# MustaphaMensouri/Distributed-Continuous-Training-with-Airflow-PyTorch-Distributed-DDP-

Measured on AMD Instinct MI355X. Metric: samples/sec (whole node) for weather-MLP DDP, higher is better.
Workload: dtype fp32; 1 GPU; global_batch=4, per_rank_batch=4, parallelism=dp1, optimizer=adam lr=0.01, loss=ce, engine=fused-persistent, dataset_rows=8649, features=5

## Files before the change

### distributed-continuous-training-with-airflow-pytorch-distributed-ddp-_amd/csrc/mlp_block5.hip

```cpp
#include "knobs.h"
#include "mlp_block5_impl.h"

namespace dct {

void mlp_launch_block5_xg(int world, size_t bytes, hipStream_t st, const MlpShape& sh, const MlpArgs& a);
void mlp_launch_block5_b8(size_t bytes, hipStream_t st, const MlpShape& sh, const MlpArgs& a);

static bool b5_xg_world_ok(int w) { return w >= 2 && w <= 8; }

bool mlp_block5_ok(const MlpShape& sh, const MlpArgs& a) {
  const bool aligned = (sh.woff[1] % 4) == 0 && ((uintptr_t)a.p & 15) == 0 && (((uintptr_t)a.m | (uintptr_t)a.v) & 15) == 0;
  const bool xg_ok = a.xg_world <= 1 ||
                     (a.mode == 0 && b5_xg_world_ok(a.xg_world) && a.xg_rank >= 0 && a.xg_rank < a.xg_world &&
                      a.xg_recv != nullptr && a.xg_peers != nullptr && a.xg_status != nullptr &&
                      (a.prof == nullptr || a.xg_world == 2 || a.xg_world == 4 || a.xg_world == 8));
  const bool b8_ok = (a.B <= blk5::B && sh.mlp_block != 8) || a.prof == nullptr;
  return aligned && b8_ok && mlp_block5_shape_ok(sh.dims, sh.L, a.B) &&
         ((a.mode == 0 && a.cursor == nullptr) || (a.mode == 1 && a.steps == 1 && a.grad_out != nullptr)) &&
         (a.loss_kind == 0 || a.loss_kind == 1) && a.pending == nullptr && (a.stage == nullptr || a.mode == 1) && xg_ok;
}

bool mlp_block5_shape_ok(const int* dims, int L, int B) {
  return L == 3 && dims[1] == blk5::H && dims[2] == blk5::H && dims[0] >= 1 && dims[0] <= blk5::DMAX &&
         dims[3] == blk5::C && B >= 1 && B <= blk5::BMAX;
}

size_t mlp_block5_xg_bytes(int world) {
  switch (world) {
    case 2: return (size_t)b5x::Lay<2>::BYTES;
    case 4: return (size_t)b5x::Lay<4>::BYTES;
    case 8: return (size_t)b5x::Lay<8>::BYTES;
    case 3: return (size_t)b5x::Lay<3>::BYTES;
    case 5: return (size_t)b5x::Lay<5>::BYTES;
    case 6: return (size_t)b5x::Lay<6>::BYTES;
    case 7: return (size_t)b5x::Lay<7>::BYTES;
    default: return 0;
  }
}

template <bool WD, int LK, bool PROF = false>
static void b5_launch_sched(int sched, size_t bytes, hipStream_t st, const MlpShape& sh, const MlpArgs& a) {
  using namespace blk5;
  if (sched == 0) return b5_launch<WD, LK, PROF>(bytes, st, sh, a);
#ifdef B5_SCHED_AB
  if constexpr (!WD && LK == 0 && !PROF) {
    constexpr int D = SCHED_DEFAULT;
    constexpr int masks[] = {D & ~SCH_PRIO_LAT, SCH_PRIO_LAT};
    bool done = false;
    b5x::static_for<sizeof(masks) / sizeof(masks[0])>([&](auto i) {
      constexpr int M = masks[decltype(i)::value];
      if (!done && sched == B5_SCHED_AB_BASE + M && M != D) {
        b5_launch<WD, LK, false, true, true, 1, -1, 1, M>(bytes, st, sh, a);
        done = true;
      }
    });
    if (done) return;
  }
#endif
  b5_launch<WD, LK, PROF, true, true, 1, -1, 1, SCHED_DEFAULT>(bytes, st, sh, a);
}

hipError_t mlp_launch_block5(const MlpShape& sh, const MlpArgs& a, hipStream_t st) {
  const size_t bytes = (size_t)blk5::LDS_FLOATS * sizeof(float);
  const bool wd = a.wd != 0.f;
  const int sched = knobs().b5_sched;
  if (a.B > blk5::B || sh.mlp_block == 8) {
    mlp_launch_block5_b8(bytes, st, sh, a);
  } else if (a.xg_world > 1) {
    mlp_launch_block5_xg(a.xg_world, bytes, st, sh, a);
  } else if (a.mode == 1) {
    if (a.loss_kind == 0) b5_launch<false, 0, false, true, false>(bytes, st, sh, a);
    else b5_launch<false, 1, false, true, false>(bytes, st, sh, a);
  } else if (a.prof) {
    if (a.loss_kind == 0) b5_launch_sched<true, 0, true>(sched, bytes, st, sh, a);
    else b5_launch_sched<true, 1, true>(sched, bytes, st, sh, a);
  } else if (a.loss_kind == 0) {
    if (wd) b5_launch_sched<true, 0>(sched, bytes, st, sh, a);
    else b5_launch_sched<false, 0>(sched, bytes, st, sh, a);
  } else {
    if (wd) b5_launch_sched<true, 1>(sched, bytes, st, sh, a);
// ... 7 lines not shown
```

### distributed-continuous-training-with-airflow-pytorch-distributed-ddp-_amd/csrc/mlp_block5_impl.h

```cpp
#pragma once
#include <type_traits>

#include "mlp_block_util.h"

namespace dct {

namespace blk5 {
constexpr int H = 128, NT = 512, NW = 8, KS = 16, DMAX = 8, B = 4, C = 2, MBMAX = 2, BMAX = B * MBMAX;
constexpr int PSTR = 36;
template <int MB>
struct Lds {
  static constexpr int RB = B * MB;
  static constexpr int XT = 0;
  static constexpr int LAB = XT + 3 * DMAX * RB;
  static constexpr int MSK = LAB + (MB == 1 ? 16 : 32);
  static constexpr int LOGP = MSK + 2 * NW * 2;
  static constexpr int H1W = LOGP + 2 * NW * 8;
  static constexpr int H1X = H1W + MB * NW * KS * 4;
  static constexpr int PART = H1X + NW * KS * 4;
  static constexpr int W2L = PART + 2 * H * PSTR;
  static constexpr int B2L = W2L + 2 * H * C;
  static constexpr int ABT = B2L + 8;
  static constexpr int TOTAL = ABT + 4;
  static_assert((H1W % 4) == 0 && (PART % 4) == 0 && (MSK % 4) == 0 && (LAB % 4) == 0 && (W2L % 4) == 0 &&
                    (B2L % 4) == 0 && (H1X % 4) == 0 && (LOGP % 4) == 0,
                "16-B aligned tiles");
};
static_assert(Lds<1>::TOTAL == 11036, "the batch <= 4 layout is round 5's");
constexpr int STG = H * H;
constexpr int LDS_FLOATS = Lds<MBMAX>::TOTAL > 2 * STG ? Lds<MBMAX>::TOTAL : 2 * STG;
static_assert(LDS_FLOATS * 4 <= 160 * 1024, "fits the CU");
using Stg = bku::Stage<H, NT>;
constexpr float LOG2E = 1.4426950408889634f, LN2 = 0.6931471805599453f;
constexpr int SCH_DROP = 1, SCH_ADAM_TAB = 2, SCH_WT1 = 8, SCH_WT2 = 16, SCH_WTB = 32;
constexpr int SCH_PRIO_LAT = 64;
constexpr int SCHED_DEFAULT = SCH_DROP | SCH_ADAM_TAB | SCH_WTB | SCH_PRIO_LAT;
}

namespace b5x {
typedef unsigned int v4u __attribute__((ext_vector_type(4)));
constexpr int SYS = 17;
constexpr int NP = 16, NS = 2;
constexpr int G = blk5::NT * 16;
template <int XW>
struct Lay {
  static constexpr int NO = (NP + XW - 1) / XW;
  static constexpr int RSS = NO + NS;
  static constexpr int AG = 2 * XW * RSS * G;
  static constexpr int LS = AG + 2 * (NP + NS) * G;
  static constexpr int EP = LS + ((2 * XW * 16 + 255) & ~255);
  static constexpr int BYTES = EP + (NP + NS) * 2 * G;
  static __device__ __forceinline__ int rs(int par, int src, int slot) { return ((par * XW + src) * RSS + slot) * G; }
  static __device__ __forceinline__ int ag(int par, int slot) { return AG + (par * (NP + NS) + slot) * G; }
  static __device__ __forceinline__ int ls(int par, int src) { return LS + (par * XW + src) * 16; }
  static __device__ __forceinline__ int ep(int slot, int mv) { return EP + (slot * 2 + mv) * G; }
};
__device__ __forceinline__ void put(__amdgpu_buffer_rsrc_t rs, int off, float x, float y, uint32_t tag) {
  v4u d;
  d.x = __float_as_uint(x);
  d.y = tag;
  d.z = __float_as_uint(y);
  d.w = tag;
  __builtin_amdgcn_raw_buffer_store_b128(d, rs, off, 0, SYS);
}
__device__ __forceinline__ bool get(__amdgpu_buffer_rsrc_t rs, int off, uint32_t tag, float& x, float& y) {
  const v4u d = __builtin_amdgcn_raw_buffer_load_b128(rs, off, 0, SYS);
  x = __uint_as_float(d.x);
  y = __uint_as_float(d.z);
  return (d.y == tag) & (d.w == tag);
// ... 13 lines not shown
    f(IC<I>{});
    static_for<N, I + 1>(f);
  }
}
}

#define B5STAMP(k)                                              \
  if constexpr (PROF) {                                         \
    const unsigned long long t_ = __builtin_amdgcn_s_memtime(); \
    pacc[(k)] += t_ - t_last;                                   \
    t_last = t_;                                                \
  }

#define B5PRIO(p)                      \
  if constexpr (S_PLAT) {              \
    __builtin_amdgcn_sched_barrier(0); \
    __builtin_amdgcn_s_setprio(p);     \
    __builtin_amdgcn_sched_barrier(0); \
  }

__device__ __forceinline__ uint32_t b5_elem(int li, int r, int u) {
  return ((uint32_t)((li * 64 + r) * 65536 + u) + 0x165667B1u) * 0xC2B2AE3Du;
}
__device__ __forceinline__ float b5_drop(uint32_t seed, uint32_t gstep, uint32_t elem, float p, float scale) {
  uint32_t h = (seed * 0x9E3779B1u) ^ ((gstep + 0x7F4A7C15u) * 0x85EBCA77u);
  h ^= elem;
  h ^= h >> 16;
  h *= 0x7feb352du;
  h ^= h >> 15;
  h *= 0x846ca68bu;
  h ^= h >> 16;
  return u01(h) < p ? 0.f : scale;
}

template <bool WD>
__device__ __forceinline__ void adam_pair(float& p0, float g0, float& m0, float& v0, float& p1, float g1, float& m1,
                                          float& v1, float b1, float b2, float wd, float A, float E) {
  if constexpr (WD) { g0 = fmaf(wd, p0, g0); g1 = fmaf(wd, p1, g1); }
  m0 = fmaf(b1, m0, g0);
  m1 = fmaf(b1, m1, g1);
  v0 = fmaf(b2, v0, g0 * g0);
  v1 = fmaf(b2, v1, g1 * g1);
  const float d0 = fmaf(__builtin_amdgcn_sqrtf(v0), A, E), d1 = fmaf(__builtin_amdgcn_sqrtf(v1), A, E);
  const float R = __builtin_amdgcn_rcpf(d0 * d1);
  p0 = fmaf(-m0, d1 * R, p0);
  p1 = fmaf(-m1, d0 * R, p1);
}

__device__ __forceinline__ bku::f32x4_t quad_transpose_mf(const float (&v)[4], const float (&e)[4]) {
  bku::f32x4_t t = (bku::f32x4_t){0.f, 0.f, 0.f, 0.f};
#pragma unroll
  for (int i = 0; i < 4; ++i) t = bku::mfma4(v[i], e[i], t);
  return t;
}

__device__ __forceinline__ float rs_bits2to5(float (&P)[16], int lane) {
  using namespace bku;
#pragma unroll
  for (int i = 0; i < 8; ++i) P[i] = swap32_sum(P[i], P[i + 8]);
#pragma unroll
  for (int i = 0; i < 4; ++i) P[i] = swap16_sum(P[i], P[i + 4]);
  const bool b3 = (lane >> 3) & 1, b2 = (lane >> 2) & 1;
#pragma unroll
  for (int i = 0; i < 2; ++i) {
    const float keep = b3 ? P[i + 2] : P[i], send = b3 ? P[i] : P[i + 2];
    P[i] = keep + dpp<ROR8>(send);
  }
  const float keep = b2 ? P[1] : P[0], send = b2 ? P[0] : P[1];
  const float t4 = dpp<ROR4>(send), t12 = dpp<0x12C>(send);
  return keep + (b2 ? t4 : t12);
}

typedef float v2f __attribute__((ext_vector_type(2)));
template <bool WD>
__device__ __forceinline__ void adam_v2(v2f& p, v2f g, v2f& m, v2f& v, float b1, float b2, float wd, float A, float E) {
  if constexpr (WD) g = (v2f)(wd) * p + g;
  m = (v2f)(b1) * m + g;
  v = (v2f)(b2) * v + g * g;
  const v2f sq = (v2f){__builtin_amdgcn_sqrtf(v.x), __builtin_amdgcn_sqrtf(v.y)};
  const v2f d = sq * (v2f)(A) + (v2f)(E);
  const float R = __builtin_amdgcn_rcpf(d.x * d.y);
  p = p - m * ((v2f){d.y, d.x} * R);
}

template <bool WD, int LK, bool PROF = false, bool DXM = true, bool ADAM = true, int XW = 1, int RK = -1, int MB = 1,
          int SCH = 0>
__global__ __launch_bounds__(blk5::NT, 1) void mlp_block5_kernel(MlpShape sh, MlpArgs a) {
  using namespace blk5;
  using namespace bku;
  static_assert(XW == 1 || (ADAM && XW >= 2 && XW <= 8), "exchange: train mode, 2..8 ranks");
  static_assert(MB >= 1 && MB <= MBMAX, "micro-batches per step");
  static_assert(SCH == 0 || (XW == 1 && MB == 1 && ADAM), "step-schedule items: one-rank train mode, one micro-batch");
  constexpr bool S_DROP = (SCH & SCH_DROP) != 0, S_TAB = (SCH & SCH_ADAM_TAB) != 0;
  constexpr int HQ = DXM ? (SCH / SCH_WT1) & 3 : 0;
  constexpr int HB = DXM ? (SCH / SCH_WTB) & 1 : 0;
  static_assert(HQ + HB <= KS / 4, "W1 has four k-blocks per wave");
  constexpr bool S_PLAT = (SCH & SCH_PRIO_LAT) != 0;
  using LY = Lds<MB>;
  constexpr int RB = LY::RB, XT = LY::XT, LAB = LY::LAB, MSK = LY::MSK, LOGP = LY::LOGP, H1W = LY::H1W;
  constexpr int H1X = LY::H1X, PART = LY::PART, W2L = LY::W2L, B2L = LY::B2L, ABT = LY::ABT, TOTAL = LY::TOTAL;
  constexpr int PS = XW > 1 ? 32 : 16;
  using XL = b5x::Lay<XW>;
  constexpr int NO = XL::NO;
  extern __shared__ __attribute__((aligned(16))) float lds[];
  const int tid = threadIdx.x, w = tid >> 6, l = tid & 63;
  const int D0 = sh.dims[0];
  const int r0 = l & 3;
  const int u = KS * w + (l >> 2);
  const int wo0 = sh.woff[0], bo0 = sh.boff[0], wo1 = sh.woff[1], bo1 = sh.boff[1];
  const int wo2 = sh.woff[2], bo2 = sh.boff[2];
  unsigned long long pacc[PROF ? PS : 1] = {};
  unsigned long long t_last = PROF ? __builtin_amdgcn_s_memtime() : 0ull;
  const unsigned long long t_kstart = t_last;

  const int Bsz = a.B;
  const int fb = tid & (RB - 1), fd = tid / RB;
  const int nel = Bsz * D0;
  int role = 0, pb = 0, pk = 0;
  if (tid < nel) { role = 1; pb = tid / D0; pk = tid - pb * D0; }
  else if (tid < nel + Bsz) { role = 2; pb = tid - nel; }
  const bool stp = !ADAM && a.stage != nullptr;
  uint32_t st_tag = 0u, st_x = 0u, st_lab = 0u;
  if (stp) {
    st_tag = a.stage[0];
    if (tid < RB * DMAX && fd < D0 && fb < Bsz) st_x = a.stage[64 + fb * D0 + fd];
    if (tid < Bsz) st_lab = a.stage[64 + nel + tid];
  }
  const int cur0 = (!ADAM && a.cursor) ? sload(a.cursor) : 0;
  const int bs0 = min(Bsz, a.n_items - cur0 * Bsz);
  const bool first_ok = tid < RB * DMAX && fb < bs0;
// ... 71 lines not shown
  if constexpr (ADAM) Stg::put(lds + STG, sm, tid);
  lds_barrier();
  if constexpr (PROF) pacc[12] = __builtin_amdgcn_s_memtime() - t_kstart;
  Stg::get<KS>(lds, w1, l, KS / 4 * w);
  if constexpr (ADAM) {
    Stg::get<KS>(lds + STG, m1, l, KS / 4 * w);
    lds_barrier();
    Stg::put(lds, sv, tid);
    lds_barrier();
    Stg::get<KS>(lds, v1, l, KS / 4 * w);
  } else {
#pragma unroll
    for (int j = 0; j < 2; ++j)
#pragma unroll
      for (int k = 0; k < KS; ++k) m1[j][k] = v1[j][k] = 0.f;
  }
  lds_barrier();
  if constexpr (PROF) pacc[13] = __builtin_amdgcn_s_memtime() - t_kstart;
  if (!ADAM && tid == 0 && cur0 > 0 && a.loss_out) a.loss_out[cur0 - 1] = a.grad_out[sh.P];

  for (int e = 4 * tid; e < TOTAL; e += 4 * NT) *reinterpret_cast<float4*>(lds + e) = make_float4(0.f, 0.f, 0.f, 0.f);
  lds_barrier();
  if (tid < RB * DMAX) lds[XT + fd * RB + fb] = x_first;
  if (tid < RB) reinterpret_cast<int*>(lds + LAB)[tid] = lab_first;
  if (own_w2) lds[W2L + u * C + r0] = r0 ? pw2[1] : pw2[0];
  if (own_b2) lds[B2L + l] = pb2;
  const uint32_t* pf_base = role == 1 ? reinterpret_cast<const uint32_t*>(a.X) + pk : reinterpret_cast<const uint32_t*>(a.Y);
  const int pf_stride = role == 1 ? a.ldx : (role == 2 ? 1 : 0);
  lds_barrier();

  if constexpr (PROF) pacc[14] = __builtin_amdgcn_s_memtime() - t_kstart;
  const float p_drop = a.dropout;
  const bool drop = p_drop > 0.f;
  const float scale = XW > 1 ? a.k_drop_scale : (drop ? 1.0f / (1.0f - p_drop) : 1.0f);
  const float l2b1 = XW > 1 ? a.k_l2b1 : log2f(a.b1), l2b2 = XW > 1 ? a.k_l2b2 : log2f(a.b2);
  const float c1 = 1.f - a.b1, c2 = 1.f - a.b2;
  const float rc1 = XW > 1 ? a.k_rc1 : 1.f / c1, rc2 = XW > 1 ? a.k_rc2 : 1.f / c2;
  const float sqc2 = XW > 1 ? a.k_sqc2 : sqrtf(c2);
#pragma unroll
  for (int j = 0; j < 2; ++j)
#pragma unroll
    for (int k = 0; k < KS; ++k) { m1[j][k] *= rc1; v1[j][k] *= rc2; }
#pragma unroll
  for (int i = 0; i < 2; ++i) { m0[i] *= rc1; v0[i] *= rc2; }
  mb0 *= rc1; vb0 *= rc2; mw2 *= rc1; vw2 *= rc2; mb1 *= rc1; vb1 *= rc2; mb2 *= rc1; vb2 *= rc2;
  mbx *= rc1; vbx *= rc2;
  v2f W[2][KS / 2], Mo[2][KS / 2], Vo[2][KS / 2];
#pragma unroll
  for (int j = 0; j < 2; ++j)
#pragma unroll
    for (int h = 0; h < KS / 2; ++h) {
      W[j][h] = (v2f){w1[j][2 * h], w1[j][2 * h + 1]};
      Mo[j][h] = (v2f){m1[j][2 * h], m1[j][2 * h + 1]};
      Vo[j][h] = (v2f){v1[j][2 * h], v1[j][2 * h + 1]};
    }
  const int xrank = XW > 1 ? (RK >= 0 ? RK : a.xg_rank) : 0;
  v2f MoO[NO], VoO[NO];
  __amdgpu_buffer_rsrc_t xrr = __builtin_amdgcn_make_buffer_rsrc((void*)a.xg_recv, 0, 0, 0x00020000), xpr[XW];
  const bool sown = XW == 1 || (__builtin_amdgcn_readfirstlane(w) % XW) == xrank;
  bool xbad = false;
  unsigned long long xticks = 0;
  if constexpr (XW > 1) {
#pragma unroll
    for (int t = 0; t < NO; ++t) {
      v2f cm[XW], cv[XW];
#pragma unroll
      for (int k = 0; k < XW; ++k) {
        const int i = XW * t + k < b5x::NP ? XW * t + k : 0;
        cm[k] = Mo[i >> 3][i & 7];
        cv[k] = Vo[i >> 3][i & 7];
      }
      MoO[t] = b5x::pick<XW>(cm, xrank);
      VoO[t] = b5x::pick<XW>(cv, xrank);
    }
  }
  if constexpr (XW > 1) {
    xrr = __builtin_amdgcn_make_buffer_rsrc((void*)a.xg_recv, 0, XL::BYTES, 0x00020000);
#pragma unroll
    for (int q = 0; q < XW; ++q)
      xpr[q] = __builtin_amdgcn_make_buffer_rsrc((void*)sload_ptr(a.xg_peers, q), 0, XL::BYTES, 0x00020000);
  }
  auto xwait = [&](uint32_t tag, auto&& sweep) -> bool {
    const unsigned long long t_start = __builtin_amdgcn_s_memrealtime();
    for (int spin = 0;; ++spin) {
      asm volatile("" ::: "memory");
      if (__all(sweep())) return true;
      if ((spin & 15) == 15 && (long long)(__builtin_amdgcn_s_memrealtime() - t_start) > a.xg_timeout) {
        if (l == 0) __hip_atomic_store(a.xg_status, tag, __ATOMIC_RELAXED, __HIP_MEMORY_SCOPE_SYSTEM);
        return false;
      }
      __builtin_amdgcn_s_sleep(1);
    }
  };
  const int tb = tid * 16;
  uint32_t el0[MB], el1[MB];
  float f1[MB], f2[MB];
#pragma unroll
  for (int hf = 0; hf < MB; ++hf) {
    el0[hf] = b5_elem(0, r0 + B * hf, u);
    el1[hf] = b5_elem(1, r0 + B * hf, u);
    f1[hf] = b5_drop(a.seed, step_base, el0[hf], p_drop, scale);
    f2[hf] = b5_drop(a.seed, step_base, el1[hf], p_drop, scale);
  }
  float* h1x = lds + H1X + w * (KS * 4);
  float eye[4];
#pragma unroll
  for (int i = 0; i < 4; ++i) eye[i] = r0 == i ? 1.f : 0.f;
  const int cb = (l >> 2) & 1;
  int xb = 0;
  float tabA = 0.f, tabE = 0.f;
  if (a.tune == 1 && w >= NW / 2) __builtin_amdgcn_s_setprio(1);
  if (a.tune == 2 && w < NW / 2) __builtin_amdgcn_s_setprio(1);
  if constexpr (PROF) {
    t_last = __builtin_amdgcn_s_memtime();
    pacc[9] = t_last - t_kstart;
  }
  for (int s = 0; s < a.steps; ++s) {
    const int sb = s + cur0;
    const int bs = min(Bsz, a.n_items - sb * Bsz);
    const uint32_t gstep = step_base + (uint32_t)s;
    const int xbn = xb == 2 ? 0 : xb + 1;
    const int pbuf = s & 1, nbuf = pbuf ^ 1;
    const float* xT = lds + XT + xb * DMAX * RB;
    const bool have_next = (s + 1 < a.steps);
    const int bs_next = have_next ? min(Bsz, a.n_items - (sb + 1) * Bsz) : 0;
    const uint32_t raw_next = pf_base[(size_t)ridx_next * pf_stride];
    const int nx2 = min((sb + 2) * Bsz + pb, a.n_items - 1);
    const int ridx_next2 = a.idx[nx2 < 0 ? 0 : nx2];
    const uint32_t xtag = gstep + 1u;
    const int xpar = (int)(gstep & 1u);
    const int t = t0 + s + 1;
    float dz2m[MB][2][4];
    float dz = 0.f, xbl = 0.f, tls = 0.f;
    float h2 = 0.f, h1 = 0.f;
    float gw0s = 0.f, gw1s = 0.f, gb1s = 0.f, gbs = 0.f, g0s = 0.f, g1s = 0.f, db0s = 0.f;
    float aA = 0.f, aE = 0.f;
    float f1n = 0.f, f2n = 0.f;
    f32x4_t wth[HQ + HB > 0 ? HQ + HB : 1][2];
    v2f GO[NO];
#pragma unroll
    for (int t2 = 0; t2 < NO; ++t2) GO[t2] = (v2f){0.f, 0.f};
    float xg_own = 0.f, xg_bx = 0.f;
    v2f xs_g0 = (v2f){0.f, 0.f}, xs_g1 = (v2f){0.f, 0.f};
    bool abort_step = false;
    auto dw1_pass = [&]() {
#pragma unroll
      for (int q = 0; q < KS / 4; ++q) {
        f32x4_t g[2];
#pragma unroll
        for (int j = 0; j < 2; ++j) g[j] = (f32x4_t){0.f, 0.f, 0.f, 0.f};
#pragma unroll
        for (int hf = 0; hf < MB; ++hf) {
          const float4 hq = *reinterpret_cast<const float4*>(lds + H1W + (hf * NW + w) * (KS * 4) + (4 * q + r0) * 4);
          const float hv[4] = {hq.x, hq.y, hq.z, hq.w};
#pragma unroll
          for (int j = 0; j < 2; ++j)
#pragma unroll
            for (int r = 0; r < 4; ++r) g[j] = mfma4(hv[r], dz2m[hf][j][r], g[j]);
        }

        if constexpr (ADAM && XW > 1) {
#pragma unroll
          for (int j = 0; j < 2; ++j)
#pragma unroll
            for (int h = 0; h < 2; ++h) {
              const int i = 8 * j + 2 * q + h;
              const float gx = g[j][2 * h], gy = g[j][2 * h + 1];
              if ((i % XW) == xrank) GO[i / XW] = (v2f){gx, gy};
              else b5x::put(xpr[i % XW], XL::rs(xpar, (xrank - i % XW + XW) % XW, i / XW) + tb, gx, gy, xtag);
            }
        } else if constexpr (ADAM) {
#pragma unroll
          for (int j = 0; j < 2; ++j)
#pragma unroll
            for (int h = 0; h < 2; ++h)
              adam_v2<WD>(W[j][2 * q + h], (v2f){g[j][2 * h], g[j][2 * h + 1]}, Mo[j][2 * q + h], Vo[j][2 * q + h], a.b1,
                          a.b2, a.wd, aA, aE);
        } else {
#pragma unroll
          for (int j = 0; j < 2; ++j)
            *reinterpret_cast<float4*>(a.grad_out + wo1 + (l + 64 * j) * H + KS * w + 4 * q) =
                make_float4(g[j][0], g[j][1], g[j][2], g[j][3]);
        }
      }
    };

#pragma unroll
    for (int hf = 0; hf < MB; ++hf) {
      const bool last = hf == MB - 1;
      const int mpar = MB == 1 ? pbuf : hf;
      float* h1w = lds + H1W + (hf * NW + w) * (KS * 4);

      const float4 xa = *reinterpret_cast<const float4*>(xT + r0 * RB + B * hf);
      const float4 xc = *reinterpret_cast<const float4*>(xT + (r0 + 4) * RB + B * hf);
      {
        const float acc0 = w0[0] * xa.x + w0[1] * xc.x, acc1 = w0[0] * xa.y + w0[1] * xc.y;
        const float acc2 = w0[0] * xa.z + w0[1] * xc.z, acc3 = w0[0] * xa.w + w0[1] * xc.w;
        const bool qb1 = (r0 >> 1) & 1, qb0 = r0 & 1;
        const float k0 = qb1 ? acc2 : acc0, k1 = qb1 ? acc3 : acc1;
        const float s0 = qb1 ? acc0 : acc2, s1 = qb1 ? acc1 : acc3;
        const float e0 = k0 + dpp<QP_X2>(s0), e1 = k1 + dpp<QP_X2>(s1);
        const float kq = qb0 ? e1 : e0, sq = qb0 ? e0 : e1;
        h1 = fmaxf(kq + dpp<QP_X1>(sq) + pb0, 0.f) * f1[hf];
        h1w[l] = h1;
        h1x[r0 * KS + (l >> 2)] = h1;
      }
      __builtin_amdgcn_wave_barrier();
      B5STAMP(0)
      {
        f32x4_t cq[2][KS / 4];
#pragma unroll
        for (int q = 0; q < KS / 4; ++q) {
          const float4 hq = *reinterpret_cast<const float4*>(h1x + r0 * KS + 4 * q);
          const float hv[4] = {hq.x, hq.y, hq.z, hq.w};
#pragma unroll
          for (int j = 0; j < 2; ++j) {
            cq[j][q] = (f32x4_t){0.f, 0.f, 0.f, 0.f};
#pragma unroll
            for (int e = 0; e < 4; ++e) cq[j][q] = mfma4(hv[e], W[j][2 * q + (e >> 1)][e & 1], cq[j][q]);
          }
        }
        f32x4_t cj[2];
#pragma unroll
        for (int j = 0; j < 2; ++j) cj[j] = (cq[j][0] + cq[j][1]) + (cq[j][2] + cq[j][3]);
        float* part = lds + PART + mpar * (H * PSTR);
#pragma unroll
        for (int j = 0; j < 2; ++j)
          *reinterpret_cast<float4*>(part + (l + 64 * j) * PSTR + w * 4) = make_float4(cj[j][0], cj[j][1], cj[j][2], cj[j][3]);
      }
      if (hf == 0) {
        if (stp) {
          const int bs_st = min(Bsz, a.n_items - (sb + 1) * Bsz);
          if (role) a.stage[64 + tid] = pb < bs_st ? raw_next : 0u;
          if (tid == 0) a.stage[0] = bs_st > 0 ? (uint32_t)(sb + 2) : 0u;
        }
        if (role) {
          const uint32_t v = (have_next && pb < bs_next) ? raw_next : 0u;
          uint32_t* dst = (role == 1) ? reinterpret_cast<uint32_t*>(lds + XT + xbn * DMAX * RB) + pk * RB + pb
                                      : reinterpret_cast<uint32_t*>(lds + LAB) + xbn * RB + pb;
          *dst = v;
        }
        ridx_next = role ? ridx_next2 : 0;
      }
      B5STAMP(1)
      lds_barrier();
      B5STAMP(2)
      B5PRIO(1)
      if constexpr (XW > 1) {
        if (lds[ABT] != 0.f) {
          abort_step = true;
          break;
        }
      }

      const float2 wv0 = *reinterpret_cast<const float2*>(lds + W2L + pbuf * (H * C) + l * C);
      const float2 wv1 = *reinterpret_cast<const float2*>(lds + W2L + pbuf * (H * C) + (l + 64) * C);
      const float b2c = lds[B2L + pbuf * 4 + cb];
      const int lab = reinterpret_cast<const int*>(lds + LAB)[xb * RB + B * hf + r0];
      {
        const float* pr = lds + PART + mpar * (H * PSTR) + u * PSTR + r0;
        float q[NW];
#pragma unroll
        for (int ww = 0; ww < NW; ++ww) q[ww] = pr[4 * ww];
        if constexpr (SCH != 0) {
          __builtin_amdgcn_sched_barrier(0);
          if constexpr (HQ > 0) {
#pragma unroll
            for (int qq = 0; qq < HQ; ++qq)
#pragma unroll
              for (int j = 0; j < 2; ++j) {
                const float wq[4] = {W[j][2 * qq].x, W[j][2 * qq].y, W[j][2 * qq + 1].x, W[j][2 * qq + 1].y};
                wth[qq][j] = quad_transpose_mf(wq, eye);
              }
          }
          if constexpr (S_DROP) {
            uint32_t gnext = gstep + 1u;
            asm volatile("" : "+s"(gnext));
            f1n = b5_drop(a.seed, gnext, el0[0], p_drop, scale);
            f2n = b5_drop(a.seed, gnext, el1[0], p_drop, scale);
            asm volatile("" : "+v"(f1n), "+v"(f2n));
          }
          if constexpr (S_TAB) {
            const int ti = s & 63;
            if (ti == 0) {
              asm volatile("");
              const float tl = (float)(t + l);
              const float step_size = a.lr * __builtin_amdgcn_rcpf(1.f - pow_t(l2b1, tl));
              const float rbc2 = __builtin_amdgcn_rsqf(1.f - pow_t(l2b2, tl));
              const float rss = __builtin_amdgcn_rcpf(step_size);
              tabA = sqc2 * rbc2 * rss * rc1;
              tabE = a.eps * rss * rc1;
            }
            aA = rl(tabA, ti);
            aE = rl(tabE, ti);
          }
          __builtin_amdgcn_sched_barrier(0);
        }
        const float z = ((q[0] + q[1]) + (q[2] + q[3])) + ((q[4] + q[5]) + (q[6] + q[7]));
        h2 = fmaxf(z + pb1, 0.f) * f2[hf];
        const float t0s = sum_bits2to5(pw2[0] * h2), t1s = sum_bits2to5(pw2[1] * h2);
        const unsigned long long msk = __ballot(h2 > 0.f);
        if (l < 8) lds[LOGP + mpar * (NW * 8) + w * 8 + l] = cb ? t1s : t0s;
        if (l == 0)
          *reinterpret_cast<uint2*>(lds + MSK + mpar * (NW * 2) + w * 2) = make_uint2((uint32_t)msk, (uint32_t)(msk >> 32));
      }
      B5STAMP(3)
      lds_barrier();
      B5STAMP(4)

      const uint2 mw0 = *reinterpret_cast<const uint2*>(lds + MSK + mpar * (NW * 2) + 2 * (l >> 4));
      const uint2 mw1 = *reinterpret_cast<const uint2*>(lds + MSK + mpar * (NW * 2) + 2 * ((l >> 4) + 4));
      float lg0 = 0.f;
      if constexpr (HB > 0) {
        lg0 = lds[LOGP + mpar * (NW * 8) + l];
        __builtin_amdgcn_sched_barrier(0);
#pragma unroll
        for (int qq = HQ; qq < HQ + HB; ++qq)
#pragma unroll
          for (int j = 0; j < 2; ++j) {
            const float wq[4] = {W[j][2 * qq].x, W[j][2 * qq].y, W[j][2 * qq + 1].x, W[j][2 * qq + 1].y};
            wth[qq][j] = quad_transpose_mf(wq, eye);
          }
        __builtin_amdgcn_sched_barrier(0);
      }
      float lv;
      {
        float lg = HB > 0 ? lg0 : lds[LOGP + mpar * (NW * 8) + l];
        lg += dpp<ROR8>(lg);
        lg = swap16_sum(lg, lg);
        lg = swap32_sum(lg, lg);
        const float z = lg + b2c;
        const float zo = dpp<ROR4>(z);
        const bool live = r0 + B * hf < bs;
        const float invb = __builtin_amdgcn_rcpf((float)(bs > 0 ? bs : 1));
        const float inv = live ? invb : 0.f;
        const float y = (cb == lab) ? 1.f : 0.f;
        if constexpr (LK == 0) {
          const float tt = zo - z;
          const float e = __builtin_amdgcn_exp2f(tt * LOG2E);
          const float pc = __builtin_amdgcn_rcpf(1.f + e);
          dz = (pc - y) * inv;
          const float sp = fmaxf(tt, 0.f) + LN2 * __builtin_amdgcn_logf(1.f + __builtin_amdgcn_exp2f(-fabsf(tt) * LOG2E));
          lv = (live && cb == lab) ? sp : 0.f;
        } else {
// ... 6 lines not shown
#pragma unroll
      for (int r = 0; r < 4; ++r)
#pragma unroll
        for (int c = 0; c < C; ++c) dz3[r][c] = rl(dz, 4 * c + r);
      if (w == 0) {
        float tl = lv + dpp<QP_X1>(lv);
        tl += dpp<QP_X2>(tl);
        tl += dpp<ROR4>(tl);
        tls = hf == 0 ? tl : tls + tl;
        if (last) {
          const float bl = bs > 0 ? tls * __builtin_amdgcn_rcpf((float)bs) : 0.f;
          if constexpr (ADAM && XW > 1) {
            xbl = rl(bl, 0);
            if (l == 0) {
#pragma unroll
              for (int q = 0; q < XW; ++q)
                if (q != xrank) b5x::put(xpr[q], XL::ls(xpar, xrank), xbl, 0.f, xtag);
            }
          } else if constexpr (ADAM) {
            if (l == 0 && a.loss_out) a.loss_out[s] = bl;
          } else {
            if (l == 0) a.grad_out[sh.P] = bl;
          }
        }
      }
      B5STAMP(5)

      if (last && !S_TAB) {
        const float step_size = a.lr * __builtin_amdgcn_rcpf(1.f - pow_t(l2b1, (float)t));
        const float rbc2 = __builtin_amdgcn_rsqf(1.f - pow_t(l2b2, (float)t));
        const float rss = __builtin_amdgcn_rcpf(step_size);
        aA = sqc2 * rbc2 * rss * rc1;
        aE = a.eps * rss * rc1;
      }
      {
        const int sh4 = 4 * (l & 15);
#pragma unroll
        for (int j = 0; j < 2; ++j) {
          const float2 wv = j ? wv1 : wv0;
          const uint2 mw = j ? mw1 : mw0;
          const uint32_t nib = ((sh4 < 32 ? mw.x : mw.y) >> (sh4 & 31)) & 15u;
#pragma unroll
          for (int r = 0; r < 4; ++r) {
            const float g = wv.x * dz3[r][0] + wv.y * dz3[r][1];
            dz2m[hf][j][r] = ((nib >> r) & 1u) ? g * scale : 0.f;
          }
        }
      }
      if constexpr (XW > 1) {
        if (last) {
          dw1_pass();
          B5STAMP(15)
        }
      }
      {
        const float d_own = dz, d_oth = dpp<ROR4>(dz);
        const float dr0 = cb ? d_oth : d_own, dr1 = cb ? d_own : d_oth;
        const float gw0 = quad_sum(dr0 * h2), gw1 = quad_sum(dr1 * h2);
        float gdz = pw2[0] * dr0 + pw2[1] * dr1;
        gdz = h2 > 0.f ? gdz * scale : 0.f;
        const float gb1 = quad_sum(gdz);
        const float gbh = (l & 1) ? (dz3[0][1] + dz3[1][1]) + (dz3[2][1] + dz3[3][1])
                                  : (dz3[0][0] + dz3[1][0]) + (dz3[2][0] + dz3[3][0]);
        gw0s = hf == 0 ? gw0 : gw0s + gw0;
        gw1s = hf == 0 ? gw1 : gw1s + gw1;
        gb1s = hf == 0 ? gb1 : gb1s + gb1;
        gbs = hf == 0 ? gbh : gbs + gbh;
        if (last) {
          float pown = (r0 & 1) ? pw2[1] : pw2[0];
          const float gown = (r0 & 1) ? gw1s : gw0s;
          const float gb = gbs;
          if constexpr (ADAM && XW > 1) {
            xg_own = gown;
            xg_bx = r0 == 1 ? gb1s : gb;
          } else if constexpr (ADAM) {
            adam_pair<WD>(pown, gown, mw2, vw2, pb1, gb1s, mb1, vb1, a.b1, a.b2, a.wd, aA, aE);
            pw2[0] = dpp<QB0>(pown);
            pw2[1] = dpp<QB1>(pown);
            if (own_w2) lds[W2L + nbuf * (H * C) + u * C + r0] = pown;
            adam_scaled<WD>(pb2, gb, mb2, vb2, a.b1, a.b2, a.wd, aA, aE);
            if (own_b2) lds[B2L + nbuf * 4 + l] = pb2;
          } else {
            if (own_w2) a.grad_out[fw2] = gown;
            if (r0 == 0) a.grad_out[bo1 + u] = gb1s;
            if (own_b2) a.grad_out[fb2] = gb;
          }
        }
      }
      B5STAMP(6)
      float dz1 = 0.f;
      if constexpr (DXM) {
        float dzt[2][4];
#pragma unroll
        for (int j = 0; j < 2; ++j) {
          const f32x4_t tq = quad_transpose_mf(dz2m[hf][j], eye);
#pragma unroll
          for (int i = 0; i < 4; ++i) dzt[j][i] = tq[i];
        }
        float P[16];
#pragma unroll
        for (int q = 0; q < KS / 4; ++q) {
          if (q == 1) B5PRIO(0)
          f32x4_t acc[2];
#pragma unroll
          for (int j = 0; j < 2; ++j) {
            const float wq[4] = {W[j][2 * q].x, W[j][2 * q].y, W[j][2 * q + 1].x, W[j][2 * q + 1].y};
            const f32x4_t wt = q < HQ + HB ? wth[q < HQ + HB ? q : 0][j] : quad_transpose_mf(wq, eye);
            acc[j] = (f32x4_t){0.f, 0.f, 0.f, 0.f};
#pragma unroll
            for (int i = 0; i < 4; ++i) acc[j] = mfma4(wt[i], dzt[j][i], acc[j]);
          }
          const f32x4_t at = acc[0] + acc[1];
#pragma unroll
// ... 7 lines not shown
#pragma unroll
          for (int kk = 0; kk < KS; ++kk)
            P[kk] = W[0][kk >> 1][kk & 1] * dz2m[hf][0][p] + W[1][kk >> 1][kk & 1] * dz2m[hf][1][p];
          const float tot = rs_small<16>(P, l);
          if (r0 == p) dz1 = tot;
        }
      }
      dz1 = h1 > 0.f ? dz1 * scale : 0.f;
      B5PRIO(1)
      {
        const float dq0 = dpp<QB0>(dz1), dq1 = dpp<QB1>(dz1), dq2 = dpp<QB2>(dz1), dq3 = dpp<QB3>(dz1);
        const float g0h = dq0 * xa.x + dq1 * xa.y + dq2 * xa.z + dq3 * xa.w;
        const float g1h = dq0 * xc.x + dq1 * xc.y + dq2 * xc.z + dq3 * xc.w;
        const float dbh = (dq0 + dq1) + (dq2 + dq3);
        g0s = hf == 0 ? g0h : g0s + g0h;
        g1s = hf == 0 ? g1h : g1s + g1h;
        db0s = hf == 0 ? dbh : db0s + dbh;
        if (last) {
          const float g0 = g0s, g1 = g1s;
          if constexpr (ADAM && XW > 1) {
            if (r0 == 0) xg_bx = db0s;
            xs_g0 = (v2f){g0, g1};
            xs_g1 = (v2f){xg_own, xg_bx};
            if (!sown) {
#pragma unroll
              for (int q = 0; q < XW; ++q)
                if (q == __builtin_amdgcn_readfirstlane(w) % XW) {
                  const int rel = (xrank - q + XW) % XW;
                  b5x::put(xpr[q], XL::rs(xpar, rel, NO) + tb, g0, g1, xtag);
                  b5x::put(xpr[q], XL::rs(xpar, rel, NO + 1) + tb, xg_own, xg_bx, xtag);
                }
            }
          } else if constexpr (ADAM) {
            adam_pair<WD>(w0[0], g0, m0[0], v0[0], w0[1], g1, m0[1], v0[1], a.b1, a.b2, a.wd, aA, aE);
            adam_scaled<WD>(pb0, db0s, mb0, vb0, a.b1, a.b2, a.wd, aA, aE);
          } else {
            if (r0 < D0) a.grad_out[wo0 + u * D0 + r0] = g0;
            if (r0 + 4 < D0) a.grad_out[wo0 + u * D0 + r0 + 4] = g1;
            if (r0 == 0) a.grad_out[bo0 + u] = db0s;
          }
        }
      }
    }
    if constexpr (XW > 1) {
      if (abort_step) break;
    }
    B5PRIO(0)
    if constexpr (S_DROP) {
      f1[0] = f1n;
      f2[0] = f2n;
    } else {
#pragma unroll
      for (int hf = 0; hf < MB; ++hf) {
        f1[hf] = b5_drop(a.seed, gstep + 1u, el0[hf], p_drop, scale);
        f2[hf] = b5_drop(a.seed, gstep + 1u, el1[hf], p_drop, scale);
      }
    }
    B5STAMP(7)
    if constexpr (XW == 1) dw1_pass();
    if constexpr (ADAM && XW > 1) {
      const unsigned long long xt0 = __builtin_amdgcn_s_memrealtime();
      const float invw = 1.f / (float)XW;
      do {
        float rv[XW][NO][2], sv[XW][2][2];
        if (!xwait(xtag, [&]() -> bool {
              bool k = true;
#pragma unroll
              for (int q = 1; q < XW; ++q)
// ... 86 lines not shown
#pragma unroll
        for (int i = 0; i < b5x::NP; ++i)
          W[i >> 3][i & 7] = (i % XW) == xrank ? WO[i / XW] : (v2f){av[i][0], av[i][1]};
        if (!sown) {
          w0[0] = sa[0][0];
          w0[1] = sa[0][1];
          xs_g1.x = sa[1][0];
          pbx = sa[1][1];
        }
        if (w == 0) {
          float tot = 0.f;
#pragma unroll
          for (int q = 0; q < XW; ++q) tot += (q == xrank) ? xbl : rl(lq, q);
          if (l == 0 && a.loss_out) a.loss_out[s] = tot * invw;
        }
      } while (false);
      if (xbad) {
        if (l == 0) lds[ABT] = 1.f;
      } else {
        const float pown = xs_g1.x;
        pw2[0] = dpp<QB0>(pown);
        pw2[1] = dpp<QB1>(pown);
        pb0 = dpp<QB0>(pbx);
        pb1 = dpp<QB1>(pbx);
        if (own_w2) lds[W2L + nbuf * (H * C) + u * C + r0] = pown;
        if (w == 0 && (l == 2 || l == 3)) lds[B2L + nbuf * 4 + (l & 1)] = pbx;
      }
      xticks += __builtin_amdgcn_s_memrealtime() - xt0;
      B5STAMP(20)
    }
    __builtin_amdgcn_wave_barrier();
    B5STAMP(8)
    xb = xbn;
  }

  if constexpr (XW > 1) {
    if (a.xg_ticks && tid == 0) atomicAdd(a.xg_ticks, xticks);
    lds_barrier();
    if (lds[ABT] != 0.f) return;
    const uint32_t etag = 0x80000000u | (step_base + (uint32_t)a.steps);
    do {
#pragma unroll
      for (int t = 0; t < NO; ++t) {
        const int o0 = XL::ep(XW * t + xrank, 0) + tb, o1 = XL::ep(XW * t + xrank, 1) + tb;
#pragma unroll
        for (int q = 0; q < XW; ++q)
          if (q != xrank && XW * t + xrank < b5x::NP) {
            b5x::put(xpr[q], o0, MoO[t].x, MoO[t].y, etag);
            b5x::put(xpr[q], o1, VoO[t].x, VoO[t].y, etag);
          }
      }
      if (sown) {
#pragma unroll
        for (int q = 0; q < XW; ++q)
          if (q != xrank) {
            b5x::put(xpr[q], XL::ep(b5x::NP, 0) + tb, m0[0], m0[1], etag);
            b5x::put(xpr[q], XL::ep(b5x::NP, 1) + tb, v0[0], v0[1], etag);
            b5x::put(xpr[q], XL::ep(b5x::NP + 1, 0) + tb, mw2, mbx, etag);
            b5x::put(xpr[q], XL::ep(b5x::NP + 1, 1) + tb, vw2, vbx, etag);
          }
      }
      float em[b5x::NP][2][2], es[2][2][2];
      const bool ok = xwait(etag, [&]() -> bool {
        bool k = true;
#pragma unroll
        for (int i = 0; i < b5x::NP; ++i) {
// ... 124 lines not shown
```

Measured before the change: 1.140 million samples/s.

## Add five micro-schedule options to block5 kernel and enable all by default

Introduces five new schedule bits that are all turned on in the default mask. Prefetch of the next batch is restricted to one wave, Adam state is packed into v2f pairs for packed updates, and the ReLU mask is stored as float factors in LDS instead of ballot bitmasks. Dropout now uses an integer threshold compare, and the b2 gradient is computed with a quad_sum plus DPP. Together these aim to trim per-step instruction count and LDS/global traffic in the fused persistent kernel, at the cost of more LDS space and some register pressure. The A/B mask list is updated so each item can be tested on its own.

Result: faster. 1.215 million samples/s (median of 6 runs) (+6.5%).

```diff
diff --git a/distributed-continuous-training-with-airflow-pytorch-distributed-ddp-_amd/csrc/mlp_block5.hip b/distributed-continuous-training-with-airflow-pytorch-distributed-ddp-_amd/csrc/mlp_block5.hip
--- a/distributed-continuous-training-with-airflow-pytorch-distributed-ddp-_amd/csrc/mlp_block5.hip
+++ b/distributed-continuous-training-with-airflow-pytorch-distributed-ddp-_amd/csrc/mlp_block5.hip
@@ -45,7 +45,9 @@
 #ifdef B5_SCHED_AB
   if constexpr (!WD && LK == 0 && !PROF) {
     constexpr int D = SCHED_DEFAULT;
-    constexpr int masks[] = {D & ~SCH_PRIO_LAT, SCH_PRIO_LAT};
+    constexpr int R = SCHED_R10;
+    constexpr int masks[] = {R, R | SCH_PF_W0, R | SCH_ADAM_SM, R | SCH_DZ2F, R | SCH_DROP_INT, R | SCH_DB2,
+                             D & ~SCH_PF_W0};
     bool done = false;
     b5x::static_for<sizeof(masks) / sizeof(masks[0])>([&](auto i) {
       constexpr int M = masks[decltype(i)::value];
diff --git a/distributed-continuous-training-with-airflow-pytorch-distributed-ddp-_amd/csrc/mlp_block5_impl.h b/distributed-continuous-training-with-airflow-pytorch-distributed-ddp-_amd/csrc/mlp_block5_impl.h
--- a/distributed-continuous-training-with-airflow-pytorch-distributed-ddp-_amd/csrc/mlp_block5_impl.h
+++ b/distributed-continuous-training-with-airflow-pytorch-distributed-ddp-_amd/csrc/mlp_block5_impl.h
@@ -22,6 +22,9 @@
   static constexpr int B2L = W2L + 2 * H * C;
   static constexpr int ABT = B2L + 8;
   static constexpr int TOTAL = ABT + 4;
+  static constexpr int DZF = TOTAL;
+  static constexpr int TOTAL_DZF = DZF + 2 * H * 4;
+  static_assert((DZF % 4) == 0, "16-B aligned");
   static_assert((H1W % 4) == 0 && (PART % 4) == 0 && (MSK % 4) == 0 && (LAB % 4) == 0 && (W2L % 4) == 0 &&
                     (B2L % 4) == 0 && (H1X % 4) == 0 && (LOGP % 4) == 0,
                 "16-B aligned tiles");
@@ -29,12 +32,16 @@
 static_assert(Lds<1>::TOTAL == 11036, "the batch <= 4 layout is round 5's");
 constexpr int STG = H * H;
 constexpr int LDS_FLOATS = Lds<MBMAX>::TOTAL > 2 * STG ? Lds<MBMAX>::TOTAL : 2 * STG;
+static_assert(Lds<1>::TOTAL_DZF <= LDS_FLOATS, "SCH_DZ2F's region inside the launch's LDS");
 static_assert(LDS_FLOATS * 4 <= 160 * 1024, "fits the CU");
 using Stg = bku::Stage<H, NT>;
 constexpr float LOG2E = 1.4426950408889634f, LN2 = 0.6931471805599453f;
 constexpr int SCH_DROP = 1, SCH_ADAM_TAB = 2, SCH_WT1 = 8, SCH_WT2 = 16, SCH_WTB = 32;
 constexpr int SCH_PRIO_LAT = 64;
-constexpr int SCHED_DEFAULT = SCH_DROP | SCH_ADAM_TAB | SCH_WTB | SCH_PRIO_LAT;
+constexpr int SCH_PF_W0 = 128, SCH_ADAM_SM = 256, SCH_DZ2F = 512, SCH_DROP_INT = 1024, SCH_DB2 = 2048;
+constexpr int SCHED_R10 = SCH_DROP | SCH_ADAM_TAB | SCH_WTB | SCH_PRIO_LAT;
+constexpr int SCHED_DEFAULT = SCHED_R10 | SCH_PF_W0 | SCH_ADAM_SM | SCH_DZ2F | SCH_DROP_INT | SCH_DB2;
+static_assert(SCHED_DEFAULT < 4096, "item masks stay below B5_SCHED_AB_BASE (knobs.h)");
 }
 
 namespace b5x {
@@ -114,6 +121,17 @@
   h ^= h >> 16;
   return u01(h) < p ? 0.f : scale;
 }
+__device__ __forceinline__ uint32_t b5_drop_thr(float p) { return (uint32_t)ceilf(p * 16777216.0f); }
+__device__ __forceinline__ float b5_drop_int(uint32_t seed, uint32_t gstep, uint32_t elem, uint32_t thr, float scale) {
+  uint32_t h = (seed * 0x9E3779B1u) ^ ((gstep + 0x7F4A7C15u) * 0x85EBCA77u);
+  h ^= elem;
+  h ^= h >> 16;
+  h *= 0x7feb352du;
+  h ^= h >> 15;
+  h *= 0x846ca68bu;
+  h ^= h >> 16;
+  return (h >> 8) < thr ? 0.f : scale;
+}
 
 template <bool WD>
 __device__ __forceinline__ void adam_pair(float& p0, float g0, float& m0, float& v0, float& p1, float g1, float& m1,
@@ -178,6 +196,8 @@
   constexpr int HB = DXM ? (SCH / SCH_WTB) & 1 : 0;
   static_assert(HQ + HB <= KS / 4, "W1 has four k-blocks per wave");
   constexpr bool S_PLAT = (SCH & SCH_PRIO_LAT) != 0;
+  constexpr bool S_PF = (SCH & SCH_PF_W0) != 0, S_SM = (SCH & SCH_ADAM_SM) != 0, S_DZF = (SCH & SCH_DZ2F) != 0;
+  constexpr bool S_DINT = (SCH & SCH_DROP_INT) != 0, S_DB2 = (SCH & SCH_DB2) != 0;
   using LY = Lds<MB>;
   constexpr int RB = LY::RB, XT = LY::XT, LAB = LY::LAB, MSK = LY::MSK, LOGP = LY::LOGP, H1W = LY::H1W;
   constexpr int H1X = LY::H1X, PART = LY::PART, W2L = LY::W2L, B2L = LY::B2L, ABT = LY::ABT, TOTAL = LY::TOTAL;
@@ -315,6 +335,7 @@
   if constexpr (PROF) pacc[14] = __builtin_amdgcn_s_memtime() - t_kstart;
   const float p_drop = a.dropout;
   const bool drop = p_drop > 0.f;
+  const uint32_t drop_thr = S_DINT ? b5_drop_thr(p_drop) : 0u;
   const float scale = XW > 1 ? a.k_drop_scale : (drop ? 1.0f / (1.0f - p_drop) : 1.0f);
   const float l2b1 = XW > 1 ? a.k_l2b1 : log2f(a.b1), l2b2 = XW > 1 ? a.k_l2b2 : log2f(a.b2);
   const float c1 = 1.f - a.b1, c2 = 1.f - a.b2;
@@ -337,6 +358,9 @@
       Mo[j][h] = (v2f){m1[j][2 * h], m1[j][2 * h + 1]};
       Vo[j][h] = (v2f){v1[j][2 * h], v1[j][2 * h + 1]};
     }
+  const v2f z2 = (v2f){0.f, 0.f};
+  v2f PSm = S_SM ? (v2f){0.f, pb1} : z2, MSm = S_SM ? (v2f){mw2, mb1} : z2, VSm = S_SM ? (v2f){vw2, vb1} : z2;
+  v2f PW0 = S_SM ? (v2f){w0[0], w0[1]} : z2, MW0 = S_SM ? (v2f){m0[0], m0[1]} : z2, VW0 = S_SM ? (v2f){v0[0], v0[1]} : z2;
   const int xrank = XW > 1 ? (RK >= 0 ? RK : a.xg_rank) : 0;
   v2f MoO[NO], VoO[NO];
   __amdgpu_buffer_rsrc_t xrr = __builtin_amdgcn_make_buffer_rsrc((void*)a.xg_recv, 0, 0, 0x00020000), xpr[XW];
@@ -385,6 +409,7 @@
     f1[hf] = b5_drop(a.seed, step_base, el0[hf], p_drop, scale);
     f2[hf] = b5_drop(a.seed, step_base, el1[hf], p_drop, scale);
   }
+  const bool pf_wave = !S_PF || __builtin_amdgcn_readfirstlane(w) == 0;
   float* h1x = lds + H1X + w * (KS * 4);
   float eye[4];
 #pragma unroll
@@ -407,9 +432,19 @@
     const float* xT = lds + XT + xb * DMAX * RB;
     const bool have_next = (s + 1 < a.steps);
     const int bs_next = have_next ? min(Bsz, a.n_items - (sb + 1) * Bsz) : 0;
-    const uint32_t raw_next = pf_base[(size_t)ridx_next * pf_stride];
-    const int nx2 = min((sb + 2) * Bsz + pb, a.n_items - 1);
-    const int ridx_next2 = a.idx[nx2 < 0 ? 0 : nx2];
+    uint32_t raw_next = 0u;
+    int ridx_next2 = 0;
+    if constexpr (S_PF) {
+      if (pf_wave) {
+        raw_next = pf_base[(size_t)(uint32_t)ridx_next * (uint32_t)pf_stride];
+        const int nx2 = min((sb + 2) * Bsz + pb, a.n_items - 1);
+        ridx_next2 = a.idx[nx2 < 0 ? 0 : nx2];
+      }
+    } else {
+      raw_next = pf_base[(size_t)ridx_next * pf_stride];
+      const int nx2 = min((sb + 2) * Bsz + pb, a.n_items - 1);
+      ridx_next2 = a.idx[nx2 < 0 ? 0 : nx2];
+    }
     const uint32_t xtag = gstep + 1u;
     const int xpar = (int)(gstep & 1u);
     const int t = t0 + s + 1;
@@ -417,7 +452,7 @@
     float dz = 0.f, xbl = 0.f, tls = 0.f;
     float h2 = 0.f, h1 = 0.f;
     float gw0s = 0.f, gw1s = 0.f, gb1s = 0.f, gbs = 0.f, g0s = 0.f, g1s = 0.f, db0s = 0.f;
-    float aA = 0.f, aE = 0.f;
+    float aA = 0.f, aE = 0.f, aEv = 0.f;
     float f1n = 0.f, f2n = 0.f;
     f32x4_t wth[HQ + HB > 0 ? HQ + HB : 1][2];
     v2f GO[NO];
@@ -477,8 +512,9 @@
       const float4 xa = *reinterpret_cast<const float4*>(xT + r0 * RB + B * hf);
       const float4 xc = *reinterpret_cast<const float4*>(xT + (r0 + 4) * RB + B * hf);
       {
-        const float acc0 = w0[0] * xa.x + w0[1] * xc.x, acc1 = w0[0] * xa.y + w0[1] * xc.y;
-        const float acc2 = w0[0] * xa.z + w0[1] * xc.z, acc3 = w0[0] * xa.w + w0[1] * xc.w;
+        const float wa = S_SM ? PW0.x : w0[0], wc = S_SM ? PW0.y : w0[1];
+        const float acc0 = wa * xa.x + wc * xc.x, acc1 = wa * xa.y + wc * xc.y;
+        const float acc2 = wa * xa.z + wc * xc.z, acc3 = wa * xa.w + wc * xc.w;
         const bool qb1 = (r0 >> 1) & 1, qb0 = r0 & 1;
         const float k0 = qb1 ? acc2 : acc0, k1 = qb1 ? acc3 : acc1;
         const float s0 = qb1 ? acc0 : acc2, s1 = qb1 ? acc1 : acc3;
@@ -517,13 +553,15 @@
           if (role) a.stage[64 + tid] = pb < bs_st ? raw_next : 0u;
           if (tid == 0) a.stage[0] = bs_st > 0 ? (uint32_t)(sb + 2) : 0u;
         }
-        if (role) {
-          const uint32_t v = (have_next && pb < bs_next) ? raw_next : 0u;
-          uint32_t* dst = (role == 1) ? reinterpret_cast<uint32_t*>(lds + XT + xbn * DMAX * RB) + pk * RB + pb
-                                      : reinterpret_cast<uint32_t*>(lds + LAB) + xbn * RB + pb;
-          *dst = v;
-        }
-        ridx_next = role ? ridx_next2 : 0;
+        if (pf_wave) {
+          if (role) {
+            const uint32_t v = (have_next && pb < bs_next) ? raw_next : 0u;
+            uint32_t* dst = (role == 1) ? reinterpret_cast<uint32_t*>(lds + XT + xbn * DMAX * RB) + pk * RB + pb
+                                        : reinterpret_cast<uint32_t*>(lds + LAB) + xbn * RB + pb;
+            *dst = v;
+          }
+          ridx_next = role ? ridx_next2 : 0;
+        }
       }
       B5STAMP(1)
       lds_barrier();
@@ -559,8 +597,13 @@
           if constexpr (S_DROP) {
             uint32_t gnext = gstep + 1u;
             asm volatile("" : "+s"(gnext));
-            f1n = b5_drop(a.seed, gnext, el0[0], p_drop, scale);
-            f2n = b5_drop(a.seed, gnext, el1[0], p_drop, scale);
+            if constexpr (S_DINT) {
+              f1n = b5_drop_int(a.seed, gnext, el0[0], drop_thr, scale);
+              f2n = b5_drop_int(a.seed, gnext, el1[0], drop_thr, scale);
+            } else {
+              f1n = b5_drop(a.seed, gnext, el0[0], p_drop, scale);
+              f2n = b5_drop(a.seed, gnext, el1[0], p_drop, scale);
+            }
             asm volatile("" : "+v"(f1n), "+v"(f2n));
           }
           if constexpr (S_TAB) {
@@ -576,23 +619,39 @@
             }
             aA = rl(tabA, ti);
             aE = rl(tabE, ti);
+            if constexpr (S_SM) {
+              aEv = aE;
+              asm volatile("" : "+v"(aEv));
+            }
           }
           __builtin_amdgcn_sched_barrier(0);
         }
         const float z = ((q[0] + q[1]) + (q[2] + q[3])) + ((q[4] + q[5]) + (q[6] + q[7]));
-        h2 = fmaxf(z + pb1, 0.f) * f2[hf];
+        h2 = fmaxf(z + (S_SM ? PSm.y : pb1), 0.f) * f2[hf];
         const float t0s = sum_bits2to5(pw2[0] * h2), t1s = sum_bits2to5(pw2[1] * h2);
-        const unsigned long long msk = __ballot(h2 > 0.f);
-        if (l < 8) lds[LOGP + mpar * (NW * 8) + w * 8 + l] = cb ? t1s : t0s;
-        if (l == 0)
-          *reinterpret_cast<uint2*>(lds + MSK + mpar * (NW * 2) + w * 2) = make_uint2((uint32_t)msk, (uint32_t)(msk >> 32));
+        if constexpr (S_DZF) {
+          lds[LY::DZF + mpar * (H * 4) + u * 4 + r0] = h2 > 0.f ? scale : 0.f;
+          if (l < 8) lds[LOGP + mpar * (NW * 8) + w * 8 + l] = cb ? t1s : t0s;
+        } else {
+          const unsigned long long msk = __ballot(h2 > 0.f);
+          if (l < 8) lds[LOGP + mpar * (NW * 8) + w * 8 + l] = cb ? t1s : t0s;
+          if (l == 0)
+            *reinterpret_cast<uint2*>(lds + MSK + mpar * (NW * 2) + w * 2) = make_uint2((uint32_t)msk, (uint32_t)(msk >> 32));
+        }
       }
       B5STAMP(3)
       lds_barrier();
       B5STAMP(4)
 
-      const uint2 mw0 = *reinterpret_cast<const uint2*>(lds + MSK + mpar * (NW * 2) + 2 * (l >> 4));
-      const uint2 mw1 = *reinterpret_cast<const uint2*>(lds + MSK + mpar * (NW * 2) + 2 * ((l >> 4) + 4));
+      uint2 mw0 = make_uint2(0u, 0u), mw1 = mw0;
+      float4 zf0 = make_float4(0.f, 0.f, 0.f, 0.f), zf1 = zf0;
+      if constexpr (S_DZF) {
+        zf0 = *reinterpret_cast<const float4*>(lds + LY::DZF + mpar * (H * 4) + l * 4);
+        zf1 = *reinterpret_cast<const float4*>(lds + LY::DZF + mpar * (H * 4) + (l + 64) * 4);
+      } else {
+        mw0 = *reinterpret_cast<const uint2*>(lds + MSK + mpar * (NW * 2) + 2 * (l >> 4));
+        mw1 = *reinterpret_cast<const uint2*>(lds + MSK + mpar * (NW * 2) + 2 * ((l >> 4) + 4));
+      }
       float lg0 = 0.f;
       if constexpr (HB > 0) {
         lg0 = lds[LOGP + mpar * (NW * 8) + l];
@@ -665,8 +724,21 @@
         const float rss = __builtin_amdgcn_rcpf(step_size);
         aA = sqc2 * rbc2 * rss * rc1;
         aE = a.eps * rss * rc1;
-      }
-      {
+        if constexpr (S_SM) aEv = aE;
+      }
+      if constexpr (S_DZF) {
+#pragma unroll
+        for (int j = 0; j < 2; ++j) {
+          const float2 wv = j ? wv1 : wv0;
+          const float4 zf = j ? zf1 : zf0;
+          const float fr[4] = {zf.x, zf.y, zf.z, zf.w};
+#pragma unroll
+          for (int r = 0; r < 4; ++r) {
+            const float g = wv.x * dz3[r][0] + wv.y * dz3[r][1];
+            dz2m[hf][j][r] = g * fr[r];
+          }
+        }
+      } else {
         const int sh4 = 4 * (l & 15);
 #pragma unroll
         for (int j = 0; j < 2; ++j) {
@@ -693,8 +765,15 @@
         float gdz = pw2[0] * dr0 + pw2[1] * dr1;
         gdz = h2 > 0.f ? gdz * scale : 0.f;
         const float gb1 = quad_sum(gdz);
-        const float gbh = (l & 1) ? (dz3[0][1] + dz3[1][1]) + (dz3[2][1] + dz3[3][1])
-                                  : (dz3[0][0] + dz3[1][0]) + (dz3[2][0] + dz3[3][0]);
+        float gbh;
+        if constexpr (S_DB2) {
+          const float qs = quad_sum(dz);
+          const float qo = dpp<0x12C>(qs);
+          gbh = (l & 1) ? qo : qs;
+        } else {
+          gbh = (l & 1) ? (dz3[0][1] + dz3[1][1]) + (dz3[2][1] + dz3[3][1])
+                        : (dz3[0][0] + dz3[1][0]) + (dz3[2][0] + dz3[3][0]);
+        }
         gw0s = hf == 0 ? gw0 : gw0s + gw0;
         gw1s = hf == 0 ? gw1 : gw1s + gw1;
         gb1s = hf == 0 ? gb1 : gb1s + gb1;
@@ -707,11 +786,17 @@
             xg_own = gown;
             xg_bx = r0 == 1 ? gb1s : gb;
           } else if constexpr (ADAM) {
-            adam_pair<WD>(pown, gown, mw2, vw2, pb1, gb1s, mb1, vb1, a.b1, a.b2, a.wd, aA, aE);
+            if constexpr (S_SM) {
+              PSm.x = pown;
+              adam_v2<WD>(PSm, (v2f){gown, gb1s}, MSm, VSm, a.b1, a.b2, a.wd, aA, aEv);
+              pown = PSm.x;
+            } else {
+              adam_pair<WD>(pown, gown, mw2, vw2, pb1, gb1s, mb1, vb1, a.b1, a.b2, a.wd, aA, aE);
+            }
             pw2[0] = dpp<QB0>(pown);
             pw2[1] = dpp<QB1>(pown);
             if (own_w2) lds[W2L + nbuf * (H * C) + u * C + r0] = pown;
-            adam_scaled<WD>(pb2, gb, mb2, vb2, a.b1, a.b2, a.wd, aA, aE);
+            adam_scaled<WD>(pb2, gb, mb2, vb2, a.b1, a.b2, a.wd, aA, S_SM ? aEv : aE);
             if (own_b2) lds[B2L + nbuf * 4 + l] = pb2;
           } else {
             if (own_w2) a.grad_out[fw2] = gown;
@@ -785,8 +870,11 @@
                 }
             }
           } else if constexpr (ADAM) {
-            adam_pair<WD>(w0[0], g0, m0[0], v0[0], w0[1], g1, m0[1], v0[1], a.b1, a.b2, a.wd, aA, aE);
-            adam_scaled<WD>(pb0, db0s, mb0, vb0, a.b1, a.b2, a.wd, aA, aE);
+            if constexpr (S_SM)
+              adam_v2<WD>(PW0, (v2f){g0, g1}, MW0, VW0, a.b1, a.b2, a.wd, aA, aEv);
+            else
+              adam_pair<WD>(w0[0], g0, m0[0], v0[0], w0[1], g1, m0[1], v0[1], a.b1, a.b2, a.wd, aA, aE);
+            adam_scaled<WD>(pb0, db0s, mb0, vb0, a.b1, a.b2, a.wd, aA, S_SM ? aEv : aE);
           } else {
             if (r0 < D0) a.grad_out[wo0 + u * D0 + r0] = g0;
             if (r0 + 4 < D0) a.grad_out[wo0 + u * D0 + r0 + 4] = g1;
@@ -939,6 +1027,10 @@
     __builtin_amdgcn_wave_barrier();
     B5STAMP(8)
     xb = xbn;
+  }
+  if constexpr (S_SM) {
+    pb1 = PSm.y; mw2 = MSm.x; mb1 = MSm.y; vw2 = VSm.x; vb1 = VSm.y;
+    w0[0] = PW0.x; w0[1] = PW0.y; m0[0] = MW0.x; m0[1] = MW0.y; v0[0] = VW0.x; v0[1] = VW0.y;
   }
 
   if constexpr (XW > 1) {
```
